# Hiroki-Maeda/ninwavelets

Hardware: AMD Instinct MI355X
Metric: CWT throughput (epochs*chans*samples*freqs)/s (higher is better)
Workload: dtype f32; 1 GPU; C4 Morse CWT, 512 epochs x 64 ch x 16384 samples x 256 freqs per GPU (4096 epochs at 8 GPUs), complex64 out; wavelet=morse, epochs=512, chans=64, samples=16384, freqs=256, output=cwt, engine=fused, chunk_signals=512, parallelism=dp1 (signals sharded, no collective)

## Files before the change

ninwavelets_amd/csrc/nw_fft_dev.h:

```cpp
#pragma once

#include <type_traits>

#include "nw_dcheck.h"
#include "nw_dft_reg.h"
#include "nw_internal.h"
#include "nw_shape.h"

#ifndef NW_PACK_MAX
#define NW_PACK_MAX 2
#endif
constexpr int kPackMax = NW_PACK_MAX;
constexpr int kPruneMin = 4;
constexpr int kXdmaMinE = 32;
constexpr int kWregMaxE = 16;

namespace nw {
namespace {


__device__ __forceinline__ C2<f2> pk(C2<float> a, C2<float> b) { return {f2{a.re, b.re}, f2{a.im, b.im}}; }
__device__ __forceinline__ C2<float> lo(C2<f2> p) { return {p.re.x, p.im.x}; }
__device__ __forceinline__ C2<float> hi(C2<f2> p) { return {p.re.y, p.im.y}; }

// ... 117 lines not shown
        const __amdgpu_buffer_rsrc_t rs = __builtin_amdgcn_make_buffer_rsrc(
            reinterpret_cast<char*>(row) + (kSoffsetInField ? 0 : c_off), 0, 0x7fffffff, 0x00020000);
        const int so = kSoffsetInField ? (int)c_off : 0;
        if constexpr (sizeof(V) == 16)
            __builtin_amdgcn_raw_buffer_store_b128(__builtin_bit_cast(__attribute__((ext_vector_type(4))) unsigned, val),
                                                   rs, (int)lane_off, so, 2);
        else if constexpr (sizeof(V) == 8)
            __builtin_amdgcn_raw_buffer_store_b64(__builtin_bit_cast(__attribute__((ext_vector_type(2))) unsigned, val),
                                                  rs, (int)lane_off, so, 2);
        else
            __builtin_amdgcn_raw_buffer_store_b32(__builtin_bit_cast(unsigned, val), rs, (int)lane_off, so, 2);
    } else {
        __builtin_nontemporal_store(val, reinterpret_cast<V*>(at(reinterpret_cast<char*>(row), lane_off, c_off)));
    }
}
template <typename O> using StoreVec =
    typename std::conditional<sizeof(O) == 16, float __attribute__((ext_vector_type(4))),
    typename std::conditional<sizeof(O) == 8, float __attribute__((ext_vector_type(2))), float>::type>::type;

template <int OUT, typename T, int SP>
__device__ __forceinline__ void store_pair(void* orow, uint32_t lane_idx, uint32_t c_idx, C2<T> y0, C2<T> y1) {
    using O = typename OutT<OUT, T>::type;
    struct alignas(2 * sizeof(O)) P2 { O a, b; };
#ifdef NW_ABL_NOSTORE
    asm volatile("" ::"v"(y0.re), "v"(y0.im), "v"(y1.re), "v"(y1.im), "v"(lane_idx));
    return;
#endif
    using V = typename std::conditional<sizeof(P2) == 16, float __attribute__((ext_vector_type(4))),
              typename std::conditional<sizeof(P2) == 8, float __attribute__((ext_vector_type(2))),
                                        double __attribute__((ext_vector_type(4)))>::type>::type;
    const P2 pv{out_value<OUT, T>(y0), out_value<OUT, T>(y1)};
    store_row<SP>(__builtin_bit_cast(V, pv), orow, lane_idx * (uint32_t)sizeof(O), c_idx * (uint32_t)sizeof(O));
}
template <int OUT, typename T, int SP>
__device__ __forceinline__ void store_one(void* orow, uint32_t lane_idx, uint32_t c_idx, C2<T> y) {
    using O = typename OutT<OUT, T>::type;
#ifdef NW_ABL_NOSTORE
    asm volatile("" ::"v"(y.re), "v"(y.im), "v"(lane_idx));
    return;
#endif
    if constexpr (SP == kStoreGlobal)
        *at(reinterpret_cast<O*>(orow), lane_idx * (uint32_t)sizeof(O), c_idx * (uint32_t)sizeof(O)) =
            out_value<OUT, T>(y);
    else
        store_row<SP>(__builtin_bit_cast(StoreVec<O>, out_value<OUT, T>(y)), orow, lane_idx * (uint32_t)sizeof(O),
                      c_idx * (uint32_t)sizeof(O));
}

#ifdef NW_STAMPS
constexpr int kStamps = 8;
__device__ unsigned long long g_nw_stamps[kStamps + 1];
struct Stamps {
    unsigned long long last, acc[kStamps];
};
__device__ __forceinline__ unsigned long long nw_now() {
    unsigned long long t;
    __builtin_amdgcn_sched_barrier(0);
    asm volatile("s_memtime %0\n\ts_waitcnt lgkmcnt(0)" : "=s"(t)::"memory");
    __builtin_amdgcn_sched_barrier(0);
    return t;
}
#define NW_STAMP(st, k)                                 \
    do {                                                \
        if (st) {    \
            const unsigned long long now_ = nw_now();   \
            (st)->acc[k] += now_ - (st)->last;          \
            (st)->last = now_;                          \
        }                                               \
    } while (0)
constexpr int kStampsStore = kStamps - 1;
#else
struct Stamps {};
#define NW_STAMP(st, k) ((void)(st))
#endif

template <typename T> struct alignas(2 * sizeof(T)) Pair {
    T a, b;
};

template <int COMP, typename T> __device__ __forceinline__ T& comp(C2<T>& c) {
    if constexpr (COMP == 0) return c.re; else return c.im;
}

template <int N, int E, int P, int OSZ = 8, bool PK = false> struct PassInfo;

template <typename T, int N, int E, int P, int COMP>
__device__ __forceinline__ void lds_write(C2<T>* v, T* lds, int t) {
    using G = Geometry<N, E>;
    constexpr int PG = kPadX<T, N, E, P + 1>;
    if constexpr (P == 0) {
        NW_DCHECK_H(lds_idx_p<PG>(t * E + E - 1) < kImgElems<T, N, E>);
        Pair<T>* dst = reinterpret_cast<Pair<T>*>(lds + lds_idx_p<PG>(t * E));
#pragma unroll
        for (int u = 0; u < E / 2; ++u)
            dst[u] = Pair<T>{comp<COMP>(v[bitrev<E>(2 * u)]), comp<COMP>(v[bitrev<E>(2 * u + 1)])};
    } else {
        constexpr int R = G::radix(P);
        constexpr int NS = G::ns(P);
        constexpr int Q = E / R;
#pragma unroll
        for (int q = 0; q < Q; ++q) {
            const int j = PassInfo<N, E, P, 16, kIsPair<T>>::bfly(t, q);
            NW_DCHECK_H(lds_idx_p<PG>((j / NS) * NS * R + j % NS) + lds_off_p<PG>((R - 1) * NS) < kImgElems<T, N, E>);
            T* dst = lds + lds_idx_p<PG>((j / NS) * NS * R + j % NS);
#pragma unroll
            for (int i = 0; i < R; ++i) dst[lds_off_p<PG>(bitrev<R>(i) * NS)] = comp<COMP>(v[q * R + i]);
        }
    }
}

template <int N, int E, int P, int OSZ, bool PK> struct PassInfo {
    using G = Geometry<N, E>;
    static constexpr int R = G::radix(P);
    static constexpr int NS = G::ns(P);
    static constexpr int Q = E / R;
    static constexpr int STRIDE = N / R;
    static constexpr bool LAST = (P == G::npass() - 1);
    static constexpr bool PAIRED = LAST && Q == 2 && OSZ <= 8;
    static_assert(STRIDE % E == 0 && NS % E == 0, "pad must stay linear");
    static constexpr bool SWZ = PAIRED && G::T == 512 && kPadG<E> == 32;
    static constexpr bool REMAP = PK && NW_PAIR_PAD16 && P == 1 && !LAST && E == 16 && G::T == 256 && Q == 1;
    __device__ static __forceinline__ int bfly(int t, int q) {
        if constexpr (SWZ) return 2 * (((t >> 5) << 4) + (((t >> 4) & 1) << 8) + (t & 15)) + q;
        if constexpr (REMAP) return ((t >> 5) << 4) + (((t >> 4) & 1) << 7) + (t & 15);
        return PAIRED ? Q * t + q : t + q * G::T;
    }
};

template <typename T, int N, int E> struct Tab1 {
    using I = PassInfo<N, E, 1>;
    using S = Sc<T>;
    static constexpr int NS = I::NS, R = I::R;
    static constexpr int COUNT = Geometry<N, E>::npass() >= 2 ? NS * (R - 1) : 0;
#ifdef NW_TAB1_F64_16384
    static constexpr bool BIG = sizeof(S) == 8 && N == 16384 && E == 32;
#else
    static constexpr bool BIG = false;
#endif
    static constexpr bool ON = COUNT > 0 && (COUNT * (int)sizeof(C2<S>) <= 8192 || BIG);
    static constexpr int BYTES = ON ? COUNT * (int)sizeof(C2<S>) : 0;
    static_assert((kImgElems<T, N, E> * sizeof(T)) % 16 == 0, "table alignment");
    __device__ static __forceinline__ const C2<S>* table(const T* lds) {
        return reinterpret_cast<const C2<S>*>(lds + kImgElems<T, N, E>);
    }
    __device__ static __forceinline__ void fill(T* lds, const C2<S>* __restrict__ tw, int t) {
        if constexpr (ON) {
            C2<S>* tab = reinterpret_cast<C2<S>*>(lds + kImgElems<T, N, E>);
            for (int i = t; i < COUNT; i += Geometry<N, E>::T) {
                const int jj = i % NS, r = i / NS + 1;
                tab[i] = tw[(jj * r * (N / (NS * R))) % N];
            }
        }
    }
};

template <typename T, int N, int E, int P, int COMP, int OSZ>
__device__ __forceinline__ void lds_read(C2<T>* v, const T* lds, int t) {
    using I = PassInfo<N, E, P, OSZ, kIsPair<T>>;
    constexpr int R = I::R, Q = I::Q;
    constexpr int PG = kPadX<T, N, E, P>;
    if constexpr (I::PAIRED) {
        NW_DCHECK_H(lds_idx_p<PG>(I::bfly(t, 0)) + (Q - 1) + lds_off_p<PG>((R - 1) * I::STRIDE) < kImgElems<T, N, E>);
        const T* src = lds + lds_idx_p<PG>(I::bfly(t, 0));
#pragma unroll
        for (int q = 0; q < Q; q += 2)
#pragma unroll
            for (int r = 0; r < R; ++r) {
                const Pair<T> pr = *reinterpret_cast<const Pair<T>*>(src + q + lds_off_p<PG>(r * I::STRIDE));
                comp<COMP>(v[q * R + r]) = pr.a;
                comp<COMP>(v[(q + 1) * R + r]) = pr.b;
            }
    } else {
#pragma unroll
        for (int q = 0; q < Q; ++q) {
            NW_DCHECK_H(lds_idx_p<PG>(I::bfly(t, q)) + lds_off_p<PG>((R - 1) * I::STRIDE) < kImgElems<T, N, E>);
            const T* src = lds + lds_idx_p<PG>(I::bfly(t, q));
#pragma unroll
            for (int r = 0; r < R; ++r) comp<COMP>(v[q * R + r]) = src[lds_off_p<PG>(r * I::STRIDE)];
        }
    }
}

__device__ __forceinline__ void lds_barrier() {
    __builtin_amdgcn_s_waitcnt(0xC07F);
    __builtin_amdgcn_s_barrier();
}

typedef __attribute__((address_space(3))) void lds_void_t;
typedef __attribute__((address_space(1))) void gbl_void_t;

template <typename T, int N, int TT>
__device__ __forceinline__ void dma_x(const C2<T>* xs, void* dst, int t, int nround = 1 << 30) {
    constexpr int CH = (N / 2) * (int)sizeof(C2<T>) / 16;
    static_assert(CH % TT == 0, "whole DMA rounds");
    const int wave_base = __builtin_amdgcn_readfirstlane((t & ~63) * 16);
    const uint32_t lane_off = (uint32_t)t * 16u;
#pragma unroll
    for (int i = 0; i < CH / TT; ++i) {
        if (i >= nround) break;
        const char* chunk = reinterpret_cast<const char*>(xs) + (size_t)i * TT * 16;
        asm volatile("" : "+s"(chunk));
        const uint32_t lds_addr = (uint32_t)(uintptr_t)(lds_void_t*)(reinterpret_cast<char*>(dst) + i * TT * 16 + wave_base);
        asm volatile("s_mov_b32 m0, %0\n\ts_nop 0\n\tglobal_load_lds_dwordx4 %1, %2"
                     :: "s"(lds_addr), "v"(lane_off), "s"(chunk) : "memory", "m0");
    }
}

__device__ __forceinline__ unsigned long long sload_u64(const void* p) {
    unsigned long long u;
    asm volatile("s_load_dwordx2 %0, %1, 0x0\n\ts_waitcnt lgkmcnt(0)" : "=s"(u) : "s"(p) : "memory");
    return u;
}
__device__ __forceinline__ C2<float> c2_of_u64(unsigned long long u) {
    return C2<float>{__uint_as_float((unsigned)u), __uint_as_float((unsigned)(u >> 32))};
}
template <typename T> __device__ __forceinline__ C2<T> sload_c2(const C2<T>* p) {
    if constexpr (sizeof(T) == 4) {
        unsigned long long u;
        asm volatile("s_load_dwordx2 %0, %1, 0x0\n\ts_waitcnt lgkmcnt(0)" : "=s"(u) : "s"(p) : "memory");
        return C2<T>{__uint_as_float((unsigned)u), __uint_as_float((unsigned)(u >> 32))};
    } else {
        typedef unsigned long long u2 __attribute__((ext_vector_type(2)));
        u2 u;
        asm volatile("s_load_dwordx4 %0, %1, 0x0\n\ts_waitcnt lgkmcnt(0)" : "=s"(u) : "s"(p) : "memory");
        return C2<T>{__longlong_as_double((long long)u.x), __longlong_as_double((long long)u.y)};
    }
}

template <int V>
__device__ __forceinline__ void wait_vmcnt() {
    static_assert(V >= 0 && V < 64, "vmcnt range");
    __builtin_amdgcn_s_waitcnt((V & 0xF) | ((V >> 4) << 14) | 0x70 | 0xF00);
}

template <int CTRL> __device__ __forceinline__ float dpp_f(float v) {
    return __int_as_float(__builtin_amdgcn_mov_dpp(__float_as_int(v), CTRL, 0xF, 0xF, false));
}
template <int CTRL> __device__ __forceinline__ double dpp_f(double v) {
    const long long b = __double_as_longlong(v);
    const int lo = __builtin_amdgcn_mov_dpp((int)(b & 0xffffffffLL), CTRL, 0xF, 0xF, false);
    const int hi = __builtin_amdgcn_mov_dpp((int)(b >> 32), CTRL, 0xF, 0xF, false);
    return __longlong_as_double(((long long)hi << 32) | (unsigned int)lo);
}
template <int D, typename F> __device__ __forceinline__ void xpose2(F& a, F& b, bool hi) {
    constexpr int CTRL = D == 1 ? 0xB1 : 0x4E;
    const F recv = dpp_f<CTRL>(hi ? a : b);
    if (hi) a = recv; else b = recv;
}
template <typename F> __device__ __forceinline__ void xpose2(C2<F>& a, C2<F>& b, bool hi, int d) {
    if (d == 1) { xpose2<1>(a.re, b.re, hi); xpose2<1>(a.im, b.im, hi); }
    else { xpose2<2>(a.re, b.re, hi); xpose2<2>(a.im, b.im, hi); }
}

template <typename T, int N, int E, int OUT, int SP = kStoreGlobal>
struct LastStores {
    using O = typename OutT<OUT, T>::type;
    using I = PassInfo<N, E, Geometry<N, E>::npass() - 1, (int)sizeof(O)>;
    static constexpr int R = I::R, Q = I::Q;
    static constexpr int STEP = I::PAIRED ? 2 : 1;
    static constexpr int PACK_W = (int)(16 / sizeof(O));
    static constexpr int PACK = (!I::PAIRED && PACK_W <= kPackMax && R % PACK_W == 0) ? PACK_W : 1;
    static_assert(PACK == 1 || PACK == 2 || PACK == 4, "pack");
    static constexpr int COUNT = PACK > 1 ? Q * R / PACK : Q / STEP * R;
    __device__ static __forceinline__ void all(const C2<T>* v, void* orow, int t) {
        if constexpr (PACK == 1) {
            chunk<0, 1>(v, orow, t);
        } else {
            const int c = t & (PACK - 1);
            const uint32_t lane = (uint32_t)((t & ~(PACK - 1)) + I::NS * c) * (uint32_t)sizeof(O);
#pragma unroll
            for (int qg = 0; qg < Q * (R / PACK); ++qg) {
                const int q = qg / (R / PACK), g = qg % (R / PACK);
                O val[PACK];
#pragma unroll
                for (int b = 0; b < PACK; ++b) val[b] = out_value<OUT, T>(v[q * R + bitrev<R>(g * PACK + b)]);
                if constexpr (PACK >= 2) {
                    const bool hi1 = c & 1;
#pragma unroll
                    for (int b = 0; b < PACK; b += 2) xpose_any<1>(val[b], val[b + 1], hi1);
                }
                if constexpr (PACK == 4) {
                    const bool hi2 = c & 2;
                    xpose_any<2>(val[0], val[2], hi2);
                    xpose_any<2>(val[1], val[3], hi2);
                }
                using V = float __attribute__((ext_vector_type(4)));
                struct alignas(16) P16 { O a[PACK]; };
                P16 pk;
#pragma unroll
                for (int b = 0; b < PACK; ++b) pk.a[b] = val[b];
#ifdef NW_ABL_NOSTORE
                asm volatile("" ::"v"(__builtin_bit_cast(V, pk)));
#else
                store_row<SP>(__builtin_bit_cast(V, pk), orow, lane,
                              (uint32_t)((q * Geometry<N, E>::T + g * PACK * I::NS) * sizeof(O)));
#endif
            }
        }
    }
    template <int D, typename F> __device__ static __forceinline__ void xpose_any(F& a, F& b, bool hi) {
        if constexpr (std::is_same<F, float>::value || std::is_same<F, double>::value) xpose2<D>(a, b, hi);
        else xpose2(a, b, hi, D);
    }
    template <int K>
    __device__ static __forceinline__ void one(const C2<T>* o, void* orow, int t) {
        constexpr int q = (K / R) * STEP, i = K % R;
        const uint32_t lane = (uint32_t)I::bfly(t, 0);
        constexpr uint32_t c = (uint32_t)((I::PAIRED ? q : q * Geometry<N, E>::T) + bitrev<R>(i) * I::NS);
        NW_DCHECK_H(lane + c + (I::PAIRED ? 1u : 0u) < (uint32_t)N);
        if constexpr (I::PAIRED)
            store_pair<OUT, T, SP>(orow, lane, c, o[q * R + i], o[(q + 1) * R + i]);
        else
            store_one<OUT, T, SP>(orow, lane, c, o[q * R + i]);
    }
    template <int C, int NCH, int K = C * COUNT / NCH>
    __device__ static __forceinline__ void chunk(const C2<T>* o, void* orow, int t) {
        if constexpr (K < (C + 1) * COUNT / NCH) {
            one<K>(o, orow, t);
            chunk<C, NCH, K + 1>(o, orow, t);
        }
    }
};



template <typename T, int E, bool REALW>
constexpr bool kXDMA = E >= (sizeof(T) == 4 ? kXdmaMinE : 32) && REALW;
template <typename T> __device__ __forceinline__ int dma_rounds_for(int nz) {
    return (nz * (int)sizeof(C2<T>) + 15) / 16;
}

template <typename T, int N, int E> struct TwSplit {
    static constexpr bool ON = std::is_same<T, double>::value && N >= 2048 && N <= 4096;
    static constexpr int NHI = N / 64, COUNT = NHI + 32;
    static constexpr int OFFSET = kImgElems<T, N, E> * (int)sizeof(T) + Tab1<T, N, E>::BYTES;
    static_assert(OFFSET % 16 == 0, "table alignment");
    static constexpr int BYTES = ON ? COUNT * (int)sizeof(C2<T>) : 0;
    __device__ static __forceinline__ const C2<T>* table(const T* lds) {
        return reinterpret_cast<const C2<T>*>(reinterpret_cast<const char*>(lds) + OFFSET);
    }
    __device__ static __forceinline__ void fill(T* lds, const C2<T>* __restrict__ tw, int t) {
        if constexpr (ON) {
            C2<T>* tab = reinterpret_cast<C2<T>*>(reinterpret_cast<char*>(lds) + OFFSET);
            for (int i = t; i < COUNT; i += Geometry<N, E>::T) tab[i] = i < NHI ? tw[i * 32] : tw[i - NHI];
        }
    }
};
template <typename T, int N, int E> constexpr int kLdsBytes =
    kImgElems<T, N, E> * (int)sizeof(T) + Tab1<T, N, E>::BYTES + TwSplit<T, N, E>::BYTES;


template <typename T, int N, int E, int OUT, int P, bool XD, int SP = kStoreGlobal>
__device__ __forceinline__ void passes_from(C2<T>* v, T* lds, int t, const C2<Sc<T>>* __restrict__ tw, C2<T>* x,
                                            const C2<T>* xs_next, void* ocur,
                                            Stamps* st, void* ocur2 = nullptr, int dma_rounds = 1 << 30,
                                            double* acc = nullptr, const void* xs_next2 = nullptr) {
    using S = Sc<T>;
    constexpr bool PAIRSIG = !std::is_same<T, S>::value;
    constexpr int OSZ = (int)sizeof(typename OutT<OUT, S>::type);
    using I = PassInfo<N, E, P, OSZ, kIsPair<T>>;
    if constexpr (P < Geometry<N, E>::npass()) {
        constexpr int R = I::R, Q = I::Q, LR = ilog2<R>();
        constexpr bool TABLED = P == 1 && Tab1<T, N, E>::ON;
        constexpr bool SPLIT = TwSplit<T, N, E>::ON;
        const C2<S>* split = nullptr;
        if constexpr (SPLIT) split = reinterpret_cast<const C2<S>*>(TwSplit<T, N, E>::table(lds));
        C2<S> pb[Q][LR > 0 ? LR : 1];
#ifndef NW_ABL_NOTWIDDLE
        if constexpr (!TABLED && I::PAIRED && Q == 2) {
            twiddle_bases<S, R, N, I::NS * R, SPLIT>(pb[0], I::bfly(t, 0) % I::NS, tw, split);
#pragma unroll
            for (int k = 0; k < LR; ++k) pb[1][k] = cmul(pb[0][k], tw[(N / (I::NS * R)) << k]);
        } else if constexpr (!TABLED) {
#pragma unroll
            for (int q = 0; q < Q; ++q) twiddle_bases<S, R, N, I::NS * R, SPLIT>(pb[q], I::bfly(t, q) % I::NS, tw, split);
        }
#endif
#ifndef NW_ABL_NOEXCH
        lds_barrier();
        lds_write<T, N, E, P - 1, 0>(v, lds, t);
        lds_barrier();
        lds_read<T, N, E, P, 0, OSZ>(v, lds, t);
        lds_barrier();
        lds_write<T, N, E, P - 1, 1>(v, lds, t);
        lds_barrier();
        lds_read<T, N, E, P, 1, OSZ>(v, lds, t);
#else
#pragma unroll
        for (int i = 0; i < E; ++i) asm volatile("" : "+v"(v[i].re), "+v"(v[i].im));
#endif
        if constexpr (I::LAST && XD) {
            if (xs_next) {
                lds_barrier();
                if constexpr (PAIRSIG) {
                    dma_x<S, N, Geometry<N, E>::T>(reinterpret_cast<const C2<S>*>(xs_next), lds, t, dma_rounds);
                    dma_x<S, N, Geometry<N, E>::T>(reinterpret_cast<const C2<S>*>(xs_next2),
                                                   reinterpret_cast<char*>(lds) + (N / 2) * sizeof(C2<S>), t, dma_rounds);
                } else {
                    dma_x<T, N, Geometry<N, E>::T>(xs_next, lds, t, dma_rounds);
                }
                __builtin_amdgcn_sched_barrier(0);
            }
        }
        NW_STAMP(st, 2 * P - 1);
#pragma unroll
        for (int q = 0; q < Q; ++q) {
#ifdef NW_ABL_NOTWIDDLE
            constexpr bool TWIDDLED = false;
#else
            constexpr bool TWIDDLED = true;
#endif
            if constexpr (std::is_same<T, float>::value && Q % 2 == 0 && !(TWIDDLED && TABLED)) {
                if (q % 2 == 0) {
                    C2<f2> pv[R];
#pragma unroll
                    for (int i = 0; i < R; ++i)
                        pv[i] = pk(reinterpret_cast<C2<float>*>(v)[q * R + i],
                                   reinterpret_cast<C2<float>*>(v)[(q + 1) * R + i]);
                    if constexpr (TWIDDLED) {
                        C2<f2> pp[LR > 0 ? LR : 1];
#pragma unroll
                        for (int k = 0; k < LR; ++k)
                            pp[k] = pk(reinterpret_cast<C2<float>*>(pb[q])[k], reinterpret_cast<C2<float>*>(pb[q + 1])[k]);
                        twiddle_dft<f2, R>(pv, pp);
                    } else {
                        idft_br<f2, R>(pv);
                    }
#pragma unroll
                    for (int i = 0; i < R; ++i) {
                        reinterpret_cast<C2<float>*>(v)[q * R + i] = lo(pv[i]);
                        reinterpret_cast<C2<float>*>(v)[(q + 1) * R + i] = hi(pv[i]);
                    }
                }
            } else if constexpr (TWIDDLED && TABLED) {
                idft_br_tw<T, R>(v + q * R, TwTable<S, R, I::NS, true>{Tab1<T, N, E>::table(lds) + I::bfly(t, q) % I::NS});
            } else if constexpr (TWIDDLED) {
                twiddle_dft<T, R>(v + q * R, pb[q]);
            } else {
                idft_br<T, R>(v + q * R);
            }
        }
        NW_STAMP(st, 2 * P);
        if constexpr (I::LAST && OUT == kOutPSum) {
            if constexpr (PAIRSIG) {
#pragma unroll
                for (int e = 0; e < Q * R; ++e) {
                    const C2<S> a{v[e].re.x, v[e].im.x};
                    acc[e] += (double)(a.re * a.re + a.im * a.im);
                }
                if (ocur2) {
#pragma unroll
                    for (int e = 0; e < Q * R; ++e) {
                        const C2<S> b{v[e].re.y, v[e].im.y};
                        acc[e] += (double)(b.re * b.re + b.im * b.im);
                    }
                }
            } else {
#pragma unroll
                for (int e = 0; e < Q * R; ++e) acc[e] += (double)(v[e].re * v[e].re + v[e].im * v[e].im);
            }
        } else if constexpr (I::LAST && OUT == kOutPhSum) {
            static_assert(!PAIRSIG, "partial sums run the single-signal kernel");
#pragma unroll
            for (int e = 0; e < Q * R; ++e) {
                const double re = (double)v[e].re, im = (double)v[e].im;
                if constexpr (sizeof(S) == 8) {
                    const double inv = 1.0 / hypot(re, im);
                    acc[2 * e] += mul_nocontract(re, inv);
                    acc[2 * e + 1] += mul_nocontract(im, inv);
// ... 59 lines not shown
```

ninwavelets_amd/csrc/nw_fused.hip:

```cpp
#include <cstdlib>
#include <map>
#include <mutex>
#include <tuple>

#define NW_TAB1_F64_16384 1
#include "nw_fft_dev.h"

namespace nw {

namespace {

template <typename T, int N, int E, int NZ = E>
__device__ __forceinline__ void load_x(C2<T>* x, const C2<T>* xs, int t) {
    constexpr int TT = N / E;
    const uint32_t xo = (uint32_t)t * (uint32_t)sizeof(C2<T>);
#pragma unroll
    for (int r = 0; r < NZ; ++r) {
        if (r < E / 2) {
            x[r] = *at(xs, xo, (uint32_t)(r * TT * sizeof(C2<T>)));
        } else {
            x[r] = *at(xs, (uint32_t)((N - r * TT) * sizeof(C2<T>)) - xo);
            x[r].im = -x[r].im;
        }
    }
}

template <typename T, bool REALW>
__device__ __forceinline__ auto wsel(cplx<T> w) {
    if constexpr (REALW) return w.re; else return C2<T>{w.re, w.im};
}

template <typename T, bool REALW> struct WLoad;
template <typename T> struct WLoad<T, true> {
    using type = T;
    __device__ static __forceinline__ C2<T> apply(T w, C2<T> x) { return {w * x.re, w * x.im}; }
};
template <typename T> struct WLoad<T, false> {
    using type = C2<T>;
    __device__ static __forceinline__ C2<T> apply(C2<T> w, C2<T> x) { return cmul(w, x); }
};

constexpr int kWKeep32 = 16, kWKeep32Small = 8;
#ifndef NW_WKEEP64
#define NW_WKEEP64 8
#endif
constexpr int kWKeep64 = NW_WKEEP64;
constexpr int kPairWKeep = 12;
constexpr int kPairWKeepRed = 10;
constexpr bool kPairXD = true;
constexpr int kWpsF32 = 4, kWpsF64 = 2, kWpsPhSum = 3, kWpsPSum32 = 2;
#ifndef NW_PRIO64
#define NW_PRIO64 1
#endif
template <typename T> constexpr bool kPrioHalf = sizeof(T) == 8 && NW_PRIO64;
__device__ __forceinline__ void prio_half(int t, int threads) {
    if (__builtin_amdgcn_readfirstlane(t) >= threads / 2) __builtin_amdgcn_s_setprio(1);
}
template <typename T, int E, int OUT>
constexpr int kWpsOf = sizeof(T) == 8 ? kWpsF64 : OUT == kOutPhSum ? kWpsPhSum
                     : (OUT == kOutPSum && E >= 32) ? kWpsPSum32 : kWpsF32;

template <typename T, int N, int E, int OUT, bool REALW, int WSH = 0>
__global__ __launch_bounds__(N / E, (kWpsOf<T, E, OUT>)) void nw_fused_kernel(WDesc d, const cplx<T>* __restrict__ X,
                                                            const void* __restrict__ wtab, void* __restrict__ out,
                                                            const C2<T>* __restrict__ tw, int64_t nsig, int group,
                                                            int nsg_pad, const int* __restrict__ wnz, int tg) {
    using G = Geometry<N, E>;
    using WT = typename WLoad<T, REALW>::type;
    constexpr bool XD = kXDMA<T, E, REALW>;
    static_assert(!XD || WSH == 0, "X LDS-DMA needs the unshifted W-support table");
    extern __shared__ __align__(16) unsigned char smem[];
    T* lds = reinterpret_cast<T*>(smem);
    const int t = threadIdx.x;
    if constexpr (kPrioHalf<T> && XD) prio_half(t, N / E);

    const BlockSlot slot = block_slot(blockIdx.x, d.nfreq, kTileFT<T>, tg);
    const int fi = slot.row, sg = slot.group;
    if (fi >= d.nfreq || sg >= nsg_pad || (int64_t)sg * group >= nsig) return;
    const int64_t s_begin = (int64_t)sg * group;
    const int64_t s_end = min(nsig, s_begin + group);

    const WT* wrow = reinterpret_cast<const WT*>(wtab) + (int64_t)fi * N;
    const uint32_t wo = (uint32_t)t * (uint32_t)sizeof(WT);
    constexpr bool WREG = E <= kWregMaxE && !(sizeof(T) == 8 && N / E > 512);
    WT w[WREG ? E : 1];
    if constexpr (WREG) {
#pragma unroll
        for (int r = 0; r < E; ++r) w[r] = *at(wrow, wo, (uint32_t)(r * G::T * sizeof(WT)));
// ... 14 lines not shown
        else return *at(wrow, wo, (uint32_t)(r * G::T * sizeof(WT)));
#endif
    };

#ifdef NW_STAMPS
    Stamps stamps{};
    Stamps* st = &stamps;
    st->last = nw_now();
#else
    Stamps* st = nullptr;
#endif
    Tab1<T, N, E>::fill(lds, tw, t);
    TwSplit<T, N, E>::fill(lds, tw, t);
    if constexpr (TwSplit<T, N, E>::ON) lds_barrier();
    C2<T> x[E];
    const int64_t out_esz = (int64_t)(OUT == NW_OUT_CWT ? sizeof(C2<T>) : sizeof(T));
    C2<T> nyq{T(0), T(0)};
    if constexpr (XD) {
        nyq = reinterpret_cast<const C2<T>*>(X + s_begin * d.nh)[N / 2];
        const int nzv0 = pass0_variant<E, kNzFineOut<T, N, E, OUT>, kNz24Of<T, N, E>>(max(1, wnz[fi] >> WSH));
        dma_x<T, N, G::T>(reinterpret_cast<const C2<T>*>(X + s_begin * d.nh),
                          lds, t, nzv0 <= E / 2 ? dma_rounds_for<T>(nzv0) : 1 << 30);
    }
    const int nz = max(1, wnz[fi] >> WSH);
    NW_DCHECK(fi < d.nfreq && s_end <= nsig && d.n == N && nz <= E);
    const int nzv = pass0_variant<E, kNzFineOut<T, N, E, OUT>, kNz24Of<T, N, E>>(nz);
    static_assert(kPruneMin == 4, "the smallest pass-0 variant");
    const int dma_rounds = nzv <= E / 2 ? dma_rounds_for<T>(nzv) : 1 << 30;
    constexpr bool PSUM = OUT == kOutPSum || OUT == kOutPhSum;
    constexpr int NACC = OUT == kOutPhSum ? 2 : 1;
    double acc[PSUM ? NACC * E : 1];
    if constexpr (PSUM) {
#pragma unroll
        for (int e = 0; e < NACC * E; ++e) acc[e] = 0.0;
    }
    for (int64_t s = s_begin; s < s_end; ++s) {
        const C2<T>* xl = nullptr;
        if constexpr (XD) {
            if (s == s_begin || PSUM) wait_vmcnt<0>(); else wait_vmcnt<LastStores<T, N, E, OUT>::COUNT>();
            lds_barrier();
            xl = reinterpret_cast<const C2<T>*>(lds);
        }
        C2<T> v[E];
        auto pass0 = [&]<int NZ>() {
            if constexpr (XD) {
                int tl = t;
                asm volatile("" : "+v"(tl));
                const C2<T>* xm = xl + (N - (E - 1) * G::T - tl);
#pragma unroll
                for (int r = 0; r < NZ; ++r) {
                    if (r < E / 2) {
                        x[r] = xl[tl + r * G::T];
                    } else {
                        x[r] = xm[(E - 1 - r) * G::T];
                        if (r == E / 2 && t == 0) x[r] = nyq;
                        x[r].im = -x[r].im;
                    }
                }
            } else {
                load_x<T, N, E, NZ>(x, reinterpret_cast<const C2<T>*>(X + s * d.nh), t);
            }
#pragma unroll
            for (int r = 0; r < E; ++r)
                v[r] = r < NZ ? WLoad<T, REALW>::apply(w_at(r), x[r]) : C2<T>{T(0), T(0)};
            idft_br<T, E, NZ>(v);
        };
        if (nzv == 4) pass0.template operator()<4>();
        else if (nzv == 8) pass0.template operator()<8>();
        else if (kNzFineOut<T, N, E, OUT> && nzv == 12) pass0.template operator()<(E > 16 ? 12 : E)>();
        else if (E > 16 && nzv == 16) pass0.template operator()<(E > 16 ? 16 : E)>();
        else if (kNzFineOut<T, N, E, OUT> && nzv == 20) pass0.template operator()<(E > 16 ? 20 : E)>();
        else if (kNz24Of<T, N, E> && nzv == 24) pass0.template operator()<(E > 16 ? 24 : E)>();
        else pass0.template operator()<E>();
        if constexpr (XD) {
            if (s + 1 < s_end) nyq = sload_c2(reinterpret_cast<const C2<T>*>(X + (s + 1) * d.nh) + N / 2);
        }
        NW_STAMP(st, 0);
        const C2<T>* xs_next = s + 1 < s_end ? reinterpret_cast<const C2<T>*>(X + (s + 1) * d.nh) : nullptr;
        void* ocur = (char*)out + (s * d.nfreq + fi) * (int64_t)N * out_esz;
        passes_from<T, N, E, OUT, 1, XD, (sizeof(T) == 8 ? kStoreGlobalNt : kStoreGlobal)>(
            v, lds, t, tw, x, xs_next, ocur, st, nullptr, dma_rounds, PSUM ? acc : nullptr);
    }
    if constexpr (PSUM) {
        using IL = PassInfo<N, E, G::npass() - 1, (int)sizeof(T)>;
        double* prow = reinterpret_cast<double*>(out) + ((int64_t)sg * d.nfreq + fi) * (int64_t)N * NACC;
#pragma unroll
        for (int q = 0; q < IL::Q; ++q)
#pragma unroll
            for (int i = 0; i < IL::R; ++i) {
                const int k = IL::bfly(t, q) + bitrev<IL::R>(i) * IL::NS, e = q * IL::R + i;
                if constexpr (NACC == 1) {
                    prow[k] = acc[e];
                } else {
                    *reinterpret_cast<double2*>(prow + 2 * k) = double2{acc[2 * e], acc[2 * e + 1]};
                }
            }
    }
    NW_STAMP(st, kStampsStore);
#ifdef NW_STAMPS
    if ((t & 63) == 0) {
        for (int k = 0; k < kStamps; ++k) atomicAdd(&g_nw_stamps[k], stamps.acc[k]);
        atomicAdd(&g_nw_stamps[kStamps], (unsigned long long)(s_end - s_begin));
    }
#endif
}

template <int N, int E, int OUT>
__global__ __launch_bounds__(N / E, (OUT == kOutXSum || OUT == kOutPlvSum) ? 2 : OUT == kOutPSum ? 3 : 4) void nw_fused_pair_kernel(WDesc d, const cplx<float>* __restrict__ X,
                                                                  const void* __restrict__ wtab, void* __restrict__ out,
                                                                  const C2<float>* __restrict__ tw, int64_t nsig,
                                                                  int group, int nsg_pad, const int* __restrict__ wnz,
                                                                  int tg) {
    using G = Geometry<N, E>;
    static_assert(E <= 16, "pair mode holds 2 x E complex values per lane");
    extern __shared__ __align__(16) unsigned char smem[];
    f2* lds = reinterpret_cast<f2*>(smem);
    const int t = threadIdx.x;
    const BlockSlot slot = block_slot(blockIdx.x, d.nfreq, kTileF, tg);
    const int fi = slot.row, sg = slot.group;
    if (fi >= d.nfreq || sg >= nsg_pad || (int64_t)sg * group >= nsig) return;
    const int64_t s_begin = (int64_t)sg * group;
    const int cnt = __builtin_amdgcn_readfirstlane((int)(min(nsig, s_begin + group) - s_begin));

    const float* wrow = reinterpret_cast<const float*>(wtab) + (int64_t)fi * N;
    const uint32_t wo = (uint32_t)t * (uint32_t)sizeof(float);
    constexpr int WK = (OUT == NW_OUT_CWT || OUT == NW_OUT_POWER ? kPairWKeep : kPairWKeepRed) < E
                           ? (OUT == NW_OUT_CWT || OUT == NW_OUT_POWER ? kPairWKeep : kPairWKeepRed) : E;
    float w[WK];
#pragma unroll
    for (int r = 0; r < WK; ++r) w[r] = *at(wrow, wo, (uint32_t)(r * G::T * sizeof(float)));
    auto w_at = [&](int r) { return r < WK ? w[r < WK ? r : 0] : *at(wrow, wo, (uint32_t)(r * G::T * sizeof(float))); };
    Tab1<f2, N, E>::fill(lds, tw, t);
    const int64_t out_esz = (int64_t)(OUT == NW_OUT_CWT ? sizeof(C2<float>) : sizeof(float));
    const int nz = wnz[fi];
    NW_DCHECK(fi < d.nfreq && s_begin + cnt <= nsig && d.n == N && nz >= 1 && nz <= E);
    auto xrow = [&](int64_t s) { return reinterpret_cast<const C2<float>*>(X + s * d.nh); };
#ifdef NW_PAIR_XD_ALL
    constexpr bool XD = kPairXD && OUT != kOutPSum;
#else
    constexpr bool XD = kPairXD && OUT == NW_OUT_CWT;
#endif
    const int nzv = nz < kPruneMin ? kPruneMin : nz;
    const int dma_rounds = nzv <= E / 2 ? dma_rounds_for<float>(nzv) : 1 << 30;
    unsigned long long nyq_a = 0, nyq_b = 0;
    if constexpr (XD) {
        const int64_t sb = cnt > 1 ? s_begin + 1 : s_begin;
        nyq_a = sload_u64(xrow(s_begin) + N / 2);
        nyq_b = sload_u64(xrow(sb) + N / 2);
        dma_x<float, N, G::T>(xrow(s_begin), lds, t, dma_rounds);
        dma_x<float, N, G::T>(xrow(sb), reinterpret_cast<char*>(lds) + (N / 2) * sizeof(C2<float>), t, dma_rounds);
    }
    constexpr bool PSUM = OUT == kOutPSum || OUT == kOutXSum || OUT == kOutPlvSum;
    constexpr int NACC = kPairAcc<OUT>;
    double acc[PSUM ? NACC * E : 1];
    if constexpr (PSUM) {
#pragma unroll
        for (int e = 0; e < NACC * E; ++e) acc[e] = 0.0;
    }
    if constexpr (NACC > 1) NW_DCHECK(cnt % 2 == 0);
    for (int i = 0; i < cnt; i += 2) {
        const int64_t s = s_begin + i;
        const bool two = i + 1 < cnt;
        const int64_t s2 = two ? s + 1 : s;
        C2<f2> v[E];
        if constexpr (XD) {
            if (i == 0) wait_vmcnt<0>(); else wait_vmcnt<2 * LastStores<float, N, E, OUT, kStoreBuffer>::COUNT>();
            lds_barrier();
// ... 421 lines not shown
```

ninwavelets_amd/csrc/nw_shape.h:

```cpp
#pragma once

#include <stddef.h>
#include <stdint.h>

#include <type_traits>

#include "../../include/ninwave.h"

#ifdef __HIP__
#define NW_SHAPE_HD __host__ __device__
#else
#define NW_SHAPE_HD
#endif
#define NW_INLINE inline __attribute__((always_inline))

namespace nw {

template <typename T> constexpr int kDtypeOf = sizeof(T) == 4 ? NW_F32 : NW_F64;


struct BlockSlot {
    int row, group;
};
NW_SHAPE_HD NW_INLINE BlockSlot block_slot(int b, int nrows, int tile_f, int tile_g) {
// ... 76 lines not shown
#define NW_TILE64_F kTileF
#endif
#ifndef NW_TILE64_G
#define NW_TILE64_G kTileG
#endif
template <typename T> constexpr int kTileFT = sizeof(T) == 8 ? NW_TILE64_F : kTileF;
template <typename T> constexpr int kTileGT = sizeof(T) == 8 ? NW_TILE64_G : kTileG;
#ifndef NW_GROUP64_16K
#define NW_GROUP64_16K 16
#endif
#ifndef NW_TILE64_G_16K
#define NW_TILE64_G_16K 2
#endif
template <typename T, int N> constexpr int kGroupOut = sizeof(T) == 8 ? (N == 16384 ? NW_GROUP64_16K : kGroup64) : kGroup;
template <typename T, int N> constexpr int kTileGOut = sizeof(T) == 8 && N == 16384 ? NW_TILE64_G_16K : kTileGT<T>;

constexpr int64_t kMinRounds = 4, kResidentBlocks = 512;
constexpr int group_filling(int base, int64_t nsig, int nfreq) {
    int g = base;
    while (g > 2 && (nsig + g - 1) / g * (int64_t)nfreq < kMinRounds * kResidentBlocks) g /= 2;
    return g;
}


constexpr size_t wtab_row_bytes(int64_t n, int nfreq, size_t esz, bool realw) {
    const size_t b = (size_t)n * nfreq * esz * (realw ? 1 : 2);
    return (b + 15) / 16 * 16;
}
inline const int* wtab_wnz(const void* wtab, int64_t n, int nfreq, size_t esz, bool realw) {
    return reinterpret_cast<const int*>(static_cast<const char*>(wtab) + wtab_row_bytes(n, nfreq, esz, realw));
}

NW_SHAPE_HD constexpr int wnz_round(int need, int e) {
    int p2 = 1;
    while (p2 < need && p2 < 8) p2 <<= 1;
    if (p2 < need) p2 = (need + 3) / 4 * 4;
    return p2 < e ? p2 : e;
}


constexpr bool kNz24 = true;
template <typename T, int N, int E> constexpr bool kNz24Of = kNz24 && E > 16;
template <typename T, int N, int E> constexpr bool kNzFineOf = kNz24Of<T, N, E> && sizeof(T) == 4;
#ifndef NW_F64_FINE
#define NW_F64_FINE 1
#endif
#if NW_F64_FINE
template <typename T, int N, int E, int OUT> constexpr bool kNzFineOut = kNzFineOf<T, N, E> ||
    (kNz24Of<T, N, E> && OUT == NW_OUT_CWT);
#else
template <typename T, int N, int E, int OUT> constexpr bool kNzFineOut = kNzFineOf<T, N, E>;
#endif
template <int E, bool FINE, bool NZ24>
NW_SHAPE_HD constexpr NW_INLINE int pass0_variant(int nz) {
    if (nz <= 4) return 4;
    if (nz <= 8) return 8;
    if (FINE && nz <= 12) return 12;
    if (E > 16 && nz <= 16) return 16;
    if (FINE && nz <= 20) return 20;
    if (NZ24 && nz <= 24) return 24;
    return E;
}
NW_SHAPE_HD constexpr int pair_pass0_variant(int nz, int e) { return nz <= 4 ? 4 : nz <= 8 ? 8 : nz <= 12 ? 12 : e; }


template <typename T, int E, bool REALW>
constexpr bool kPairMode = std::is_same<T, float>::value && E <= 16 && REALW;

template <typename T, int EO, bool PHASE>
constexpr int kPsE = (EO >= 32 && (PHASE || sizeof(T) == 8)) ? 16 : EO;
template <int EO, int E> constexpr int kPsShift = EO == E ? 0 : EO == 2 * E ? 1 : 2;
template <typename T, int N, int EO>
constexpr bool kPSumOK = !(sizeof(T) == 8 && N / kPsE<T, EO, false> > 512);
template <typename T, int N, int EO>
constexpr bool kPhSumOK = N / kPsE<T, EO, true> <= 512;

template <int N> constexpr bool kPairXSumOK = N >= 1024 && N <= 4096;
template <int N> constexpr bool kPairPlvSumOK = N >= 1024 && N <= 4096;
constexpr bool pair_partials_supported(int64_t n, int dtype, int kind, int out_kind) {
    if (dtype != NW_F32 || (kind != NW_MORSE && kind != NW_MORLET && kind != NW_SHANNON)) return false;
    const bool xs = n == 1024 ? kPairXSumOK<1024> : n == 2048 ? kPairXSumOK<2048> : n == 4096 ? kPairXSumOK<4096> : false;
    const bool ps = n == 1024 ? kPairPlvSumOK<1024> : n == 2048 ? kPairPlvSumOK<2048> : n == 4096 ? kPairPlvSumOK<4096> : false;
    return out_kind == NW_OUT_CROSS_SUM ? xs : out_kind == NW_OUT_PLV_SUM ? ps : false;
}


constexpr int kConnPairs = 64;
constexpr int kConnCh = 16;
constexpr int kConnTileN = 64;
constexpr int kConnWaves = 4;
constexpr int kConnPerWave = kConnPairs / kConnWaves;
static_assert(kConnPairs % kConnWaves == 0 && kConnCh % kConnWaves == 0, "conn geometry");
struct ConnTile {
    int32_t nch, npairs;
    int32_t ch[kConnCh];
    int32_t sa[kConnPairs], sb[kConnPairs], out[kConnPairs];
};
struct ConnSlot {
    int64_t unit;
    int tile;
};
NW_SHAPE_HD NW_INLINE ConnSlot conn_slot(int64_t b, int ntiles, bool xcd) {
    if (!xcd) return {b / ntiles, (int)(b % ntiles)};
    const int64_t local = b >> 3;
    return {(local / ntiles) * 8 + (b & 7), (int)(local % ntiles)};
}
constexpr int64_t conn_units(int nfreq, int64_t n_out) { return (int64_t)nfreq * ((n_out + kConnTileN - 1) / kConnTileN); }
constexpr int64_t conn_blocks(int64_t nunits, int ntiles, bool xcd) {
    return (xcd ? (nunits + 7) / 8 * 8 : nunits) * ntiles;
}


constexpr int kLargeLog2Min = 15, kLargeLog2Max = 24;
constexpr bool large_supported(int64_t n, int dtype) {
    return (dtype == NW_F32 || dtype == NW_F64) && n >= (int64_t(1) << kLargeLog2Min) &&
           n <= (int64_t(1) << kLargeLog2Max) && !(n & (n - 1));
}

constexpr int kMaxN2 = 16384;
struct Split {
    int n1, n2;
};
constexpr Split large_split(int64_t n) {
    const int64_t n1 = n / kMaxN2 > 32 ? n / kMaxN2 : 32;
    return {(int)n1, (int)(n / n1)};
}

template <typename T, int N1, int N2> struct LargeSplit {};
template <typename T, int LG, typename R, typename F>
inline R for_large_length(int64_t n, R miss, F& f) {
    if constexpr (LG > kLargeLog2Max) {
        return miss;
    } else {
        constexpr Split sp = large_split(int64_t(1) << LG);
        if (n == (int64_t(1) << LG)) return f(LargeSplit<T, sp.n1, sp.n2>{});
        return for_large_length<T, LG + 1>(n, miss, f);
    }
}
template <typename R, typename F>
inline R for_large_split(int64_t n, int dtype, R miss, F f) {
    if (dtype == NW_F32) return for_large_length<float, kLargeLog2Min>(n, miss, f);
    if (dtype == NW_F64) return for_large_length<double, kLargeLog2Min>(n, miss, f);
    return miss;
}

template <typename T, int N2> constexpr int kRowE = N2 >= 8192 ? 32 : 16;
template <typename T, int N2> constexpr int kRowETab = sizeof(T) == 8 ? 16 : kRowE<T, N2>;
constexpr int kRowGroup = 4;
constexpr int row_group_of(int nf) { return nf < kRowTileF ? 1 : kRowGroup; }
NW_SHAPE_HD constexpr NW_INLINE int row_need(int km, int k1, int n1, int threads) {
    return km < k1 ? 1 : (km - k1) / n1 / threads + 1;
}
template <typename T, int E, bool TABLE> constexpr bool kRowFine = E > 16 && sizeof(T) == 4 && !TABLE;
template <typename T, int E, bool TABLE> constexpr bool kRowXD = sizeof(T) == 4 && E >= 32 && !TABLE;
template <int E> constexpr int kRowLdsNz = E / 2;

#ifdef NW_COLS64_E16
template <typename T> constexpr int kColThreads = 1024;
#else
template <typename T> constexpr int kColThreads = sizeof(T) == 8 ? 512 : 1024;
#endif
#ifdef NW_COLS64_E16
template <typename T> constexpr int kColE = sizeof(T) == 4 ? 32 : 16;
#else
template <typename T> constexpr int kColE = 32;
#endif
// ... 91 lines not shown
```

Baseline: 654.6 billion points/s.

## Use lane-indexed LDS image with ds_write_addtid stores for fp32 n=16384 exchanges

Adds a new LDS data layout for the fp32 N=16384, E=32 FFT exchanges between passes 0-1 and 1-2. Writes use ds_write_addtid_b32 with an M0 base per wave and immediate offsets, so per-lane address arithmetic is dropped. Reads use matching base and offset formulas with strides 513 and 544 chosen to avoid bank conflicts. The goal is fewer VALU address instructions and fewer LDS bank conflicts during transposes, at the cost of inline asm that requires EXEC to be all ones and a layout that must keep two blocks per CU within the LDS budget.

```diff
diff --git a/ninwavelets_amd/csrc/nw_fft_dev.h b/ninwavelets_amd/csrc/nw_fft_dev.h
--- a/ninwavelets_amd/csrc/nw_fft_dev.h
+++ b/ninwavelets_amd/csrc/nw_fft_dev.h
@@ -223,13 +223,75 @@
     if constexpr (COMP == 0) return c.re; else return c.im;
 }
 
-template <int N, int E, int P, int OSZ = 8, bool PK = false> struct PassInfo;
+template <int N, int E, int P, int OSZ = 8, bool PK = false, bool LN = false> struct PassInfo;
+typedef __attribute__((address_space(3))) void lds_void_t;
+
+#ifdef NW_LANE_IMAGE_TU
+constexpr bool kLaneImageTU = true;
+#else
+constexpr bool kLaneImageTU = false;
+#endif
+template <typename T, int N, int E, int OUT>
+constexpr bool kLaneImage = kLaneImageTU && kLaneImageShape<T, N, E> && OUT != kOutXHalf;
+
+template <int OFF0, int STEP, bool WAIT>
+__device__ __forceinline__ void addtid_store16(uint32_t m0, const float* d) {
+    static_assert(OFF0 >= 0 && OFF0 + 15 * STEP < 65536, "16-bit offset field");
+    asm volatile(
+        "s_mov_b32 m0, %16\n\ts_nop 0\n\t"
+        "ds_write_addtid_b32 %0 offset:%17+0*%18\n\t"
+        "ds_write_addtid_b32 %1 offset:%17+1*%18\n\t"
+        "ds_write_addtid_b32 %2 offset:%17+2*%18\n\t"
+        "ds_write_addtid_b32 %3 offset:%17+3*%18\n\t"
+        "ds_write_addtid_b32 %4 offset:%17+4*%18\n\t"
+        "ds_write_addtid_b32 %5 offset:%17+5*%18\n\t"
+        "ds_write_addtid_b32 %6 offset:%17+6*%18\n\t"
+        "ds_write_addtid_b32 %7 offset:%17+7*%18\n\t"
+        "ds_write_addtid_b32 %8 offset:%17+8*%18\n\t"
+        "ds_write_addtid_b32 %9 offset:%17+9*%18\n\t"
+        "ds_write_addtid_b32 %10 offset:%17+10*%18\n\t"
+        "ds_write_addtid_b32 %11 offset:%17+11*%18\n\t"
+        "ds_write_addtid_b32 %12 offset:%17+12*%18\n\t"
+        "ds_write_addtid_b32 %13 offset:%17+13*%18\n\t"
+        "ds_write_addtid_b32 %14 offset:%17+14*%18\n\t"
+        "ds_write_addtid_b32 %15 offset:%17+15*%18"
+        :: "v"(d[0]), "v"(d[1]), "v"(d[2]), "v"(d[3]), "v"(d[4]), "v"(d[5]), "v"(d[6]), "v"(d[7]),
+           "v"(d[8]), "v"(d[9]), "v"(d[10]), "v"(d[11]), "v"(d[12]), "v"(d[13]), "v"(d[14]), "v"(d[15]),
+           "s"(m0), "i"(OFF0), "i"(STEP)
+        : "memory", "m0");
+    if constexpr (WAIT) asm volatile("s_waitcnt lgkmcnt(0)" ::: "memory");
+}
 
 template <typename T, int N, int E, int P, int COMP>
+__device__ __forceinline__ void lane_write(C2<T>* v, T* lds, int t) {
+    namespace L = lane_image;
+    static_assert(kLaneImageShape<T, N, E> && (P == 0 || P == 1), "the fp32 n = 16384 exchanges");
+    static_assert(Geometry<N, E>::T % 64 == 0 && Geometry<N, E>::T == L::kT && L::kRebias == 16,
+                  "whole waves (EXEC all ones), 16 stores per M0");
+    static_assert(L::kElems <= kImgElems<T, N, E>, "the padded images' region holds these");
+    NW_DCHECK_H(__builtin_amdgcn_read_exec() == ~0ull);
+    const uint32_t img = (uint32_t)(uintptr_t)(lds_void_t*)lds;
+    const int wave = __builtin_amdgcn_readfirstlane(t >> 6);
+    float d[E];
+#pragma unroll
+    for (int k = 0; k < E; ++k) d[k] = comp<COMP>(v[bitrev<E>(k)]);
+    if constexpr (P == 0) {
+        addtid_store16<L::off_01(0), L::off_01(1) - L::off_01(0), false>(img + L::m0_01(wave), d);
+        addtid_store16<L::off_01(16), L::off_01(1) - L::off_01(0), true>(img + L::m0_01(wave), d + 16);
+    } else {
+        static_assert(PassInfo<N, E, P, 16>::R == E && PassInfo<N, E, P, 16>::Q == 1, "one radix-E butterfly per thread");
+        addtid_store16<L::off_12(0), L::off_12(1) - L::off_12(0), false>(img + L::m0_12(wave, 0), d);
+        addtid_store16<L::off_12(16), L::off_12(17) - L::off_12(16), true>(img + L::m0_12(wave, 16), d + 16);
+    }
+}
+
+template <typename T, int N, int E, int P, int COMP, bool LN = false>
 __device__ __forceinline__ void lds_write(C2<T>* v, T* lds, int t) {
     using G = Geometry<N, E>;
     constexpr int PG = kPadX<T, N, E, P + 1>;
-    if constexpr (P == 0) {
+    if constexpr (LN) {
+        lane_write<T, N, E, P, COMP>(v, lds, t);
+    } else if constexpr (P == 0) {
         NW_DCHECK_H(lds_idx_p<PG>(t * E + E - 1) < kImgElems<T, N, E>);
         Pair<T>* dst = reinterpret_cast<Pair<T>*>(lds + lds_idx_p<PG>(t * E));
 #pragma unroll
@@ -250,7 +312,7 @@
     }
 }
 
-template <int N, int E, int P, int OSZ, bool PK> struct PassInfo {
+template <int N, int E, int P, int OSZ, bool PK, bool LN> struct PassInfo {
     using G = Geometry<N, E>;
     static constexpr int R = G::radix(P);
     static constexpr int NS = G::ns(P);
@@ -259,7 +321,7 @@
     static constexpr bool LAST = (P == G::npass() - 1);
     static constexpr bool PAIRED = LAST && Q == 2 && OSZ <= 8;
     static_assert(STRIDE % E == 0 && NS % E == 0, "pad must stay linear");
-    static constexpr bool SWZ = PAIRED && G::T == 512 && kPadG<E> == 32;
+    static constexpr bool SWZ = PAIRED && G::T == 512 && kPadG<E> == 32 && !LN;
     static constexpr bool REMAP = PK && NW_PAIR_PAD16 && P == 1 && !LAST && E == 16 && G::T == 256 && Q == 1;
     __device__ static __forceinline__ int bfly(int t, int q) {
         if constexpr (SWZ) return 2 * (((t >> 5) << 4) + (((t >> 4) & 1) << 8) + (t & 15)) + q;
@@ -295,12 +357,29 @@
     }
 };
 
-template <typename T, int N, int E, int P, int COMP, int OSZ>
+template <typename T, int N, int E, int P, int COMP, int OSZ, bool LN = false>
 __device__ __forceinline__ void lds_read(C2<T>* v, const T* lds, int t) {
-    using I = PassInfo<N, E, P, OSZ, kIsPair<T>>;
+    using I = PassInfo<N, E, P, OSZ, kIsPair<T>, LN>;
     constexpr int R = I::R, Q = I::Q;
     constexpr int PG = kPadX<T, N, E, P>;
-    if constexpr (I::PAIRED) {
+    if constexpr (LN) {
+        namespace L = lane_image;
+        if constexpr (P == 1) {
+            static_assert(Q == 1 && R == E && !I::PAIRED, "pass 1: butterfly t, slots t + 512 r");
+            const T* src = lds + L::rbase_01(I::bfly(t, 0));
+#pragma unroll
+            for (int r = 0; r < R; ++r) comp<COMP>(v[r]) = src[L::roff_01(r)];
+        } else {
+            static_assert(P == 2 && Q == 2 && I::PAIRED && I::STRIDE == 1024, "pass 2: pairs 2t, 2t + 1, slots j2 + 1024 r");
+            const T* src = lds + L::rbase_12(I::bfly(t, 0));
+#pragma unroll
+            for (int r = 0; r < R; ++r) {
+                const Pair<T> pr = *reinterpret_cast<const Pair<T>*>(src + L::roff_12(r));
+                comp<COMP>(v[r]) = pr.a;
+                comp<COMP>(v[R + r]) = pr.b;
+            }
+        }
+    } else if constexpr (I::PAIRED) {
         NW_DCHECK_H(lds_idx_p<PG>(I::bfly(t, 0)) + (Q - 1) + lds_off_p<PG>((R - 1) * I::STRIDE) < kImgElems<T, N, E>);
         const T* src = lds + lds_idx_p<PG>(I::bfly(t, 0));
 #pragma unroll
@@ -327,7 +406,6 @@
     __builtin_amdgcn_s_barrier();
 }
 
-typedef __attribute__((address_space(3))) void lds_void_t;
 typedef __attribute__((address_space(1))) void gbl_void_t;
 
 template <typename T, int N, int TT>
@@ -396,7 +474,7 @@
 template <typename T, int N, int E, int OUT, int SP = kStoreGlobal>
 struct LastStores {
     using O = typename OutT<OUT, T>::type;
-    using I = PassInfo<N, E, Geometry<N, E>::npass() - 1, (int)sizeof(O)>;
+    using I = PassInfo<N, E, Geometry<N, E>::npass() - 1, (int)sizeof(O), false, kLaneImage<T, N, E, OUT>>;
     static constexpr int R = I::R, Q = I::Q;
     static constexpr int STEP = I::PAIRED ? 2 : 1;
     static constexpr int PACK_W = (int)(16 / sizeof(O));
@@ -499,7 +577,8 @@
     using S = Sc<T>;
     constexpr bool PAIRSIG = !std::is_same<T, S>::value;
     constexpr int OSZ = (int)sizeof(typename OutT<OUT, S>::type);
-    using I = PassInfo<N, E, P, OSZ, kIsPair<T>>;
+    constexpr bool LN = kLaneImage<T, N, E, OUT>;
+    using I = PassInfo<N, E, P, OSZ, kIsPair<T>, LN>;
     if constexpr (P < Geometry<N, E>::npass()) {
         constexpr int R = I::R, Q = I::Q, LR = ilog2<R>();
         constexpr bool TABLED = P == 1 && Tab1<T, N, E>::ON;
@@ -519,13 +598,13 @@
 #endif
 #ifndef NW_ABL_NOEXCH
         lds_barrier();
-        lds_write<T, N, E, P - 1, 0>(v, lds, t);
+        lds_write<T, N, E, P - 1, 0, LN>(v, lds, t);
         lds_barrier();
-        lds_read<T, N, E, P, 0, OSZ>(v, lds, t);
+        lds_read<T, N, E, P, 0, OSZ, LN>(v, lds, t);
         lds_barrier();
-        lds_write<T, N, E, P - 1, 1>(v, lds, t);
+        lds_write<T, N, E, P - 1, 1, LN>(v, lds, t);
         lds_barrier();
-        lds_read<T, N, E, P, 1, OSZ>(v, lds, t);
+        lds_read<T, N, E, P, 1, OSZ, LN>(v, lds, t);
 #else
 #pragma unroll
         for (int i = 0; i < E; ++i) asm volatile("" : "+v"(v[i].re), "+v"(v[i].im));
diff --git a/ninwavelets_amd/csrc/nw_fused.hip b/ninwavelets_amd/csrc/nw_fused.hip
--- a/ninwavelets_amd/csrc/nw_fused.hip
+++ b/ninwavelets_amd/csrc/nw_fused.hip
@@ -4,6 +4,7 @@
 #include <tuple>
 
 #define NW_TAB1_F64_16384 1
+#define NW_LANE_IMAGE_TU 1
 #include "nw_fft_dev.h"
 
 namespace nw {
@@ -184,7 +185,7 @@
             v, lds, t, tw, x, xs_next, ocur, st, nullptr, dma_rounds, PSUM ? acc : nullptr);
     }
     if constexpr (PSUM) {
-        using IL = PassInfo<N, E, G::npass() - 1, (int)sizeof(T)>;
+        using IL = PassInfo<N, E, G::npass() - 1, (int)sizeof(T), false, kLaneImage<T, N, E, OUT>>;
         double* prow = reinterpret_cast<double*>(out) + ((int64_t)sg * d.nfreq + fi) * (int64_t)N * NACC;
 #pragma unroll
         for (int q = 0; q < IL::Q; ++q)
diff --git a/ninwavelets_amd/csrc/nw_shape.h b/ninwavelets_amd/csrc/nw_shape.h
--- a/ninwavelets_amd/csrc/nw_shape.h
+++ b/ninwavelets_amd/csrc/nw_shape.h
@@ -182,6 +182,35 @@
     const bool xs = n == 1024 ? kPairXSumOK<1024> : n == 2048 ? kPairXSumOK<2048> : n == 4096 ? kPairXSumOK<4096> : false;
     const bool ps = n == 1024 ? kPairPlvSumOK<1024> : n == 2048 ? kPairPlvSumOK<2048> : n == 4096 ? kPairPlvSumOK<4096> : false;
     return out_kind == NW_OUT_CROSS_SUM ? xs : out_kind == NW_OUT_PLV_SUM ? ps : false;
+}
+
+
+#ifndef NW_LANE_IMAGE
+#define NW_LANE_IMAGE 1
+#endif
+template <typename T, int N, int E>
+constexpr bool kLaneImageShape = NW_LANE_IMAGE && std::is_same<T, float>::value && N == 16384 && E == 32;
+namespace lane_image {
+constexpr int kN = 16384, kE = 32, kT = kN / kE;
+constexpr int kS1 = 513, kS2 = 544;
+constexpr int kElems = kE * kS2;
+constexpr int kBytes = kElems * 4;
+constexpr int kTab1Bytes = kE * (kE - 1) * 8;
+constexpr int kCuLdsBytes = 160 * 1024;
+constexpr int kRebias = 16;
+NW_SHAPE_HD constexpr int addr01(int i) { return (i % kE) * kS1 + i / kE; }
+NW_SHAPE_HD constexpr int addr12(int i) { return ((i % 1024) / 32) * kS2 + (i / 1024) * 32 + i % 32; }
+NW_SHAPE_HD constexpr int m0_01(int wave) { return 256 * wave; }
+NW_SHAPE_HD constexpr int off_01(int p) { return 4 * p * kS1; }
+NW_SHAPE_HD constexpr int m0_12(int wave, int ip) { return 256 * wave + (ip >= kRebias ? 4 * kRebias * kS2 : 0); }
+NW_SHAPE_HD constexpr int off_12(int ip) { return 4 * (ip % kRebias) * kS2; }
+NW_SHAPE_HD constexpr int rbase_01(int u) { return (u % kE) * kS1 + u / kE; }
+NW_SHAPE_HD constexpr int roff_01(int r) { return (kT / kE) * r; }
+NW_SHAPE_HD constexpr int rbase_12(int j2) { return (j2 / 32) * kS2 + j2 % 32; }
+NW_SHAPE_HD constexpr int roff_12(int r) { return 32 * r; }
+static_assert(addr01(kN - 1) < kElems && addr12(kN - 1) < kElems, "both images inside the region");
+static_assert(off_01(kE - 1) < 65536 && off_12(kE - 1) < 65536, "16-bit offset field");
+static_assert(2 * (kBytes + kTab1Bytes) <= kCuLdsBytes, "two blocks per CU");
 }
 
 
```

Result: faster. 664.4 billion points/s, median of 6 (+1.5%).
